# Autonomous-Drone-Racing-Lab/Efficient-Path-Planner

Hardware: AMD Instinct MI355X
Metric: validity checks/sec + full plan ms/track, 1/2/4/8 MI355X vs CPU ref (higher is better)
Workload: dtype f64; 1 GPU; C2: 1 track, 8 gates, 64 OBBs, 1,048,576 sampled states per step; obbs=64, can_pass_gate=False, parallelism=replicas x1 (independent samplers), process_group=solo, launch=hip graph of the K steps

## Files before the change

### efficient-path-planner_amd/csrc/epp_internal.h

```cpp
#pragma once
#include <math.h>
#include <stdint.h>

#include <mutex>
#include <shared_mutex>
#include <string>
#include <vector>

#include <hip/hip_runtime_api.h>

#include "epp.h"

namespace epp {
epp_status generate_trajectory_into(const double* wp, int32_t n_wp, const double* times, double v_max,
                                    double a_max, double dt, double t0, const double v0[3], const double a0[3],
                                    double* (*alloc)(void*, int64_t), void* ctx, int64_t* n_rows);
struct FusedCheck {
    const epp_world* world;
    const double* xyz;
    int64_t n;
    double min_distance;
    uint8_t* valid;
};
epp_status check_and_generate_into(const FusedCheck* chk, const double* wp, int32_t n_wp, const double* times,
// ... 20 lines not shown
                       int32_t* radj, uint16_t* radj16, void* stream);
epp_status check_knn_motions_rows(const epp_world* world, const double* nodes, int32_t* rows32, const int32_t* ids32,
                                  const int64_t* rows_n, int32_t cap, int32_t k, int32_t can_pass_gate,
                                  uint8_t* valid, uint16_t* out16, int32_t target, int64_t* count, void* stream,
                                  const MotionMask* marks = nullptr);
bool knn_motions_rows_supported(const epp_world* world);

struct PlanSeg {
    uint64_t seed;
    double s[3], g[3];
    double bound;
    double gbound;
    double glo[3], ghi[3];
    double h;
    int64_t row_off;
    int64_t need_off;
    int32_t cap;
    int32_t need_cap;
};
enum : int { kPbRows = 1, kPbPerSeg = 3 };
struct PlanBatchLayout {
    int32_t S = 0, k = 0, ns_log = 0, nbc = 0, cap_total = 0, nctr = 0;
    int64_t ns = 0, NS = 0, need_cap = 0;
    size_t o_seg = 0, o_ctr = 0, o_xyz = 0, o_valid = 0, o_nodes = 0, o_cstat = 0, o_kws = 0, kws_stride = 0,
           o_query = 0, o_ids32 = 0, o_rows32 = 0, o_rows16 = 0, o_ev = 0, o_mark = 0, o_map = 0, o_nstat = 0,
           o_need = 0, dev_bytes = 0;
    size_t h_seg = 0, h_hdr = 0, h_slot = 0, h_rows = 0, h_need = 0, h_done = 0, host_bytes = 0;
    int32_t done_n = 0;
};
PlanBatchLayout plan_batch_layout(int32_t S, int64_t ns, int32_t k, PlanSeg* segs);
void plan_batch_trace_print();
epp_status plan_batch_launch(const epp_world* world, int32_t can_pass_gate, const double lo[3], const double hi[3],
                             const PlanBatchLayout& L, void* dev, void* host, uint32_t seq, void* stream);
}

namespace epp {

enum Field : int {
    F_LOX = 0, F_LOY, F_LOZ, F_HIX, F_HIY, F_HIZ,
    F_CX, F_CY, F_CZ,
    F_COS, F_SIN,
    F_HX, F_HY, F_HZ,
    EPP_NF
};

constexpr int kRecDoubles = 17;
constexpr int R_META = 16;

constexpr int kPtDoubles = 16;
constexpr int P_TX = F_HX, P_TY = F_HY, P_TZ = F_HZ;
#if defined(__HIPCC__)
__host__ __device__
#endif
constexpr uint32_t pt_chunk_off(uint32_t i, uint32_t c) { return (i << 7) + ((c ^ ((i >> 1) & 7u)) << 4); }
constexpr uint32_t kIdFill = 0x8000u;

// ... 143 lines not shown
```

### efficient-path-planner_amd/csrc/host_plan_solve.cpp

```cpp
#include <atomic>
#include <chrono>
#include <condition_variable>
#include <cstdlib>
#include <cstring>
#include <deque>
#include <exception>
#include <functional>
#include <iostream>
#include <mutex>
#include <thread>

#include <hip/hip_runtime_api.h>
#include <immintrin.h>

#include "completion.h"
#include "graph_search.h"
#include "host_scratch.h"
#include "plan_solve.h"

namespace epp {

namespace {
using Clock = std::chrono::steady_clock;
double ms_between(Clock::time_point a, Clock::time_point b) { return std::chrono::duration<double, std::milli>(b - a).count(); }
// ... 44 lines not shown
        if (dev) epp_free(dev);
        dev = nullptr;
        cap = 0;
        check(epp_malloc(&dev, bytes), what);
        cap = bytes;
    }
    void ensure(size_t dev_bytes, size_t host_bytes) {
        if (dev_bytes > dcap_) regrow(dev_, dcap_, std::max(dev_bytes, dcap_ + dcap_ / 2), "planner batch workspace");
        if (host_bytes > host_.cap &&
            host_.grow(std::max(host_bytes, host_.cap + host_.cap / 2), true) != hipSuccess)
            throw std::runtime_error("planner batch: hipHostMalloc failed");
    }
    void* dev() const { return dev_; }
    char* host() const { return host_.as<char>(); }
    uint32_t next_seq() { return epp::next_seq(seq_); }
    struct Area {
        void* dev = nullptr;
        PinnedBuf pin;
        void* stream = nullptr;
        size_t dcap = 0;
        bool cold = true;
    };
    static size_t r256(size_t b) { return (b + 255) & ~size_t(255); }
    static size_t area_dev_bytes(int64_t n, int k) {
        const size_t m = (size_t)n * k;
        return r256(16) + r256(m * 4) + r256(m * 2) + r256(m) + r256((size_t)epp_knn_workspace_size((int32_t)n)) +
               3 * r256((size_t)(n + 1) * 4) + r256(m * 4) + r256(m * 2);
    }
    static size_t area_pin_bytes(int64_t n, int k) {
        return r256(64) + r256((size_t)n * 24) + r256((size_t)n * k * 4) + r256((size_t)(n + 1) * 4) +
               r256((size_t)n * k * 4);
    }
    void ensure_areas(size_t W, int64_t n, int k) {
        if (areas_.size() < W) areas_.resize(W);
        const size_t db = area_dev_bytes(n, k), pb = area_pin_bytes(n, k);
        for (size_t w = 0; w < W; ++w) {
            Area& a = areas_[w];
            if (!a.stream) check(epp_stream_create(&a.stream), "stream");
            if (db > a.dcap) regrow(a.dev, a.dcap, db, "planner fallback workspace");
            if (pb > a.pin.cap) {
                if (a.pin.grow(pb) != hipSuccess) throw std::runtime_error("planner fallback: hipHostMalloc failed");
                check(epp_memcpy_d2h_async(a.pin.p, a.dev, std::min(pb, a.dcap), a.stream), "planner fallback warm-up");
                check(epp_stream_sync(a.stream), "planner fallback warm-up");
            }
        }
    }
    Area& area(size_t w) { return areas_[w]; }
    void* stream() {
        if (!stream_) check(epp_stream_create(&stream_), "stream");
        return stream_;
    }
    ~BatchScratch() {
        if (dev_) epp_free(dev_);
        if (stream_) epp_stream_destroy(stream_);
        for (Area& a : areas_) {
            if (a.dev) epp_free(a.dev);
            if (a.stream) epp_stream_destroy(a.stream);
        }
// ... 29 lines not shown
        rev.fill.assign(16384, 0);
        rev.radj.assign((size_t)16384 * k, 0);
        ss.begin(16384);
        ss.heap.resize(ss.heap.capacity() / 4);
        ss.heap.clear();
    }
};

bool plan_trace() {
    static const bool t = [] {
        const char* e = std::getenv("EPP_PLAN_TRACE");
        return e && std::atoi(e) == 1;
    }();
    return t;
}

class WholeTable {
public:
    struct Counts {
        int64_t kept, into_goal;
    };
    WholeTable(const PlanContext& c, BatchScratch::Area& a, ProblemOut& o) : c_(c), a_(a), o_(o) {}

    void enqueue(const double* d_nodes, int32_t n, const double box[6], bool want_counts = false) {
        t0_ = mark_ = Clock::now();
        const int k = c_.k;
        d_nodes_ = d_nodes;
        n_ = n;
        m_ = (size_t)n * k;
        narrow_ = n <= 65535;
        const size_t ws_bytes = (size_t)epp_knn_workspace_size(n);
        if (BatchScratch::area_dev_bytes(n, k) > a_.dcap || BatchScratch::area_pin_bytes(n, k) > a_.pin.cap)
            throw std::runtime_error("planPath: fallback workspace too small");
        char* dp = static_cast<char*>(a_.dev);
        d_ecnt_ = reinterpret_cast<int64_t*>(dp);
        d_nbr_ = reinterpret_cast<int32_t*>(dp + r256(16));
        d_nbr16_ = narrow_ ? reinterpret_cast<uint16_t*>(reinterpret_cast<char*>(d_nbr_) + r256(m_ * 4)) : nullptr;
        uint8_t* d_ev = reinterpret_cast<uint8_t*>(d_nbr_) + r256(m_ * 4) + r256(m_ * 2);
        d_ws_ = d_ev + r256(m_);
        void* st = a_.stream;
        if (hipMemsetAsync(d_ecnt_, 0, 16, static_cast<hipStream_t>(st)) != hipSuccess)
            throw std::runtime_error("planPath: clearing the edge counts failed");
        check(epp_knn_ws_box(d_nodes, n, k, 0.0, box, box + 3, d_nbr_, d_ws_, ws_bytes, st), "knn");
        const int32_t cp = c_.canPass ? 1 : 0;
        const epp_status ks = check_knn_motions_masked(c_.world, d_nodes, d_nbr_, n, k, cp, d_ev, d_nbr16_, 1, d_ecnt_, st);
        if (ks == EPP_ERR_UNSUPPORTED) {
            ThreadScratch& ts = ThreadScratch::get();
            ts.reset(2 * ThreadScratch::rounded(m_ * 24));
            double* d_e1 = static_cast<double*>(ts.carve(m_ * 24));
            double* d_e2 = static_cast<double*>(ts.carve(m_ * 24));
            check(epp_knn_edges(d_nodes, d_nbr_, n, k, d_e1, d_e2, st), "edges");
            check(epp_check_motions(c_.world, d_e1, d_e2, (int64_t)m_, cp, 0, d_ev, st), "motion check");
            check(mask_edges_count_acc(d_nbr_, d_ev, (int64_t)m_, 1, d_ecnt_, st, d_nbr16_), "mask edges");
        } else {
            check(ks, "motion check");
        }
        if (want_counts) check(epp_memcpy_d2h_async(ecnt(), d_ecnt_, 16, st), "download");
// ... 93 lines not shown

struct Emitted {
    const uint64_t* hdr;
    const uint32_t* slots;
    const uint16_t* rows;
    const double* need;
    std::vector<int64_t> first;
    int S, k;
    const double* d_nodes0;
    size_t node_stride;
    int64_t hv(int field, int p) const { return (int64_t)hdr[kPbPerSeg + field * S + p]; }
    const double* d_nodes(int p) const { return d_nodes0 + (size_t)p * node_stride * 3; }
};

int rows_symmetrised(SolveScratch& sc, const Rows& g, double bound, ProblemOut& o) {
    sc.rev.build(g);
    const Searched s = search_rows(sc.ss, g, NodePos{sc.ndc.data()}, bound, &sc.rev);
    o.pops += s.pops;
    o.why = s.r == -1 ? 5 : s.r == 0 ? 6 : -1;
    o.symmetrised = s.r == 1 ? 1 : 0;
    return s.r;
}

void census(int p, double bound, const Rows& g, WholeTable& wt, ProblemOut& o) {
    SolveScratch& sc = SolveScratch::get();
    o.fallback = 1;
    o.why = 2;
    const auto ts0 = Clock::now();
    const int r2 = rows_symmetrised(sc, g, bound, o);
    if (plan_trace())
        std::cerr << "[plan trace] problem " << p << ": symmetrised search on " << o.restricted_rows << " rows / "
                  << g.m << " nodes: " << o.pops << " closed, " << ms_between(ts0, Clock::now()) << " ms, result " << r2
                  << " (copies before: " << o.ms_restricted << " ms)" << std::endl;
    const WholeTable::Counts cnt = wt.counts();
    if (cnt.into_goal > 0) o.why = 2;
    if (cnt.into_goal == 0 && r2 == 1) {
        o.path = extract_path(sc.ss, NodePos{sc.ndc.data()});
        o.found = true;
        o.fallback = 0;
        o.census = 1;
        o.rows_down = o.restricted_rows;
    } else {
        o.found = wt.search(o.path);
        o.rows_down = o.n;
        o.symmetrised = 0;
    }
}

void solve_problem(const Emitted& em, int p, const PlanSeg& seg, const double* kbox, WholeTable& wt, ProblemOut& o) {
    const int k = em.k;
    const int64_t n = em.hv(3, p);
    o.n = n;
    const int64_t packed = em.hv(0, p);
    const int64_t m = std::min<int64_t>(em.hv(4, p), seg.need_cap);
    const auto t0 = Clock::now();
    int r = 0;
    if (seg.cap > 0) o.why = (n > 65535 || packed > seg.cap || m < 2) ? 0 : em.hv(5, p) != 0 ? 1 : -1;
    if (seg.cap > 0 && n <= 65535 && packed <= seg.cap && em.hv(5, p) == 0 && m >= 2) {
        const int64_t first = em.first[p], nrow = em.first[p + 1] - first;
        SolveScratch& sc = SolveScratch::get();
        grow_to(sc.ndc, (size_t)m * 3, 3 * 16384);
        grow_to(sc.rowc, (size_t)nrow * k, (size_t)16384 * k);
        std::memcpy(sc.ndc.data(), em.need + 3 * seg.need_off, (size_t)m * 24);
        std::memcpy(sc.rowc.data(), em.rows + (size_t)first * k, (size_t)nrow * k * 2);
        o.ms_copy = ms_between(t0, Clock::now());
        grow_to(sc.row_of, (size_t)m, 16384);
        std::fill(sc.row_of.begin(), sc.row_of.begin() + m, -1);
        for (int64_t sl = 0; sl < nrow; ++sl) sc.row_of[em.slots[first + sl] & 0xFFFFu] = (int32_t)sl;
        const Rows g{sc.rowc.data(), sc.row_of.data(), k, m};
        const NodePos pos{sc.ndc.data()};
        const bool goal_edges = em.hv(2, p) > 0;
        const Searched fwd = goal_edges ? search_rows(sc.ss, g, pos, seg.bound) : Searched{-1, 0};
        r = fwd.r;
        o.restricted_rows = packed;
        o.pops = fwd.pops;
        o.nodes = m;
        o.why = r == -1 ? 3 : r == 0 ? 4 : -1;
        if (r == 0) {
            r = rows_symmetrised(sc, g, seg.bound, o);
        } else if (!goal_edges) {
            o.ms_restricted = ms_between(t0, Clock::now());
            o.ms_search += o.ms_restricted;
            wt.enqueue(em.d_nodes(p), (int32_t)n, kbox, true);
            census(p, seg.bound, g, wt, o);
            return;
        }
        if (r == 1) {
            o.path = extract_path(sc.ss, pos);
            o.found = true;
            o.edges_checked = packed * k;
            o.edges_valid = em.hv(1, p);
            o.rows_down = packed;
        }
    }
    o.ms_restricted = ms_between(t0, Clock::now());
    o.ms_search += o.ms_restricted;
    if (r != 1) {
        o.fallback = seg.cap > 0 ? 1 : 0;
        wt.enqueue(em.d_nodes(p), (int32_t)n, kbox);
        o.found = wt.search(o.path);
        o.rows_down += n;
    }
}

template <class Solve>
class SolveCrew {
public:
    SolveCrew(size_t W, int S, int k, Solve& solve) : S_(S), k_(k), solve_(solve), err_(S), pending_(W - 1) {
        int devno = 0;
        if (hipGetDevice(&devno) != hipSuccess) devno = 0;
        for (size_t t = 1; t < W; ++t) plan_pool().submit([this, devno, t] { wait_then_drain(devno, t); });
    }
    ~SolveCrew() {
        if (go_.load(std::memory_order_acquire) == 0) set_go(-1);
        join();
    }
    void run() {
        set_go(1);
        drain(0);
        join();
        for (const auto& e : err_)
            if (e) std::rethrow_exception(e);
    }

// ... 79 lines not shown
    const size_t W = std::min((size_t)S, (size_t)std::max(1, c.threads));
    bs.ensure_areas(W, nmax, k);
    char* H = bs.host();
    std::memcpy(H + L.h_seg, segs.data(), sizeof(PlanSeg) * S);
    Emitted em{reinterpret_cast<const uint64_t*>(H + L.h_hdr), reinterpret_cast<const uint32_t*>(H + L.h_slot),
               reinterpret_cast<const uint16_t*>(H + L.h_rows), reinterpret_cast<const double*>(H + L.h_need),
               std::vector<int64_t>(S + 1, 0), S, k,
               reinterpret_cast<const double*>(static_cast<const char*>(bs.dev()) + L.o_nodes), (size_t)L.NS};
    BatchSolution sol;
    sol.out.resize(S);
    auto solve = [&](int p, size_t w) {
        WholeTable wt(c, bs.area(w), sol.out[p]);
        solve_problem(em, p, segs[p], kbox[p].data(), wt, sol.out[p]);
    };
    SolveCrew<decltype(solve)> crew(W, S, k, solve);
    sol.ms_enqueue = launch_and_wait(c, L, bs, t0);
    for (int p = 0; p < S; ++p) em.first[p + 1] = em.first[p] + std::min<int64_t>(em.hv(0, p), segs[p].cap);
    for (size_t a = 0; a < W; ++a) {
        BatchScratch::Area& ar = bs.area(a);
        if (!ar.cold) continue;
        ar.cold = false;
        ProblemOut unused;
        WholeTable wt(c, ar, unused);
        wt.enqueue(em.d_nodes(0), (int32_t)em.hv(3, 0), kbox[0].data());
        (void)wt.search(unused.path);
    }
    sol.ms_batch = ms_between(t0, Clock::now());
    crew.run();
    return sol;
}

}
```

### efficient-path-planner_amd/csrc/plan_batch.hip

```cpp
#include <hip/hip_runtime.h>

#include <algorithm>
#include <cstdio>
#include <cstdlib>
#include <string>

#include "completion.h"
#include "epp_internal.h"
#include "knn_grid.h"

namespace epp {
namespace {

constexpr int kPbSegSmall = 16;
struct PlanBatchDev {
    const PlanSeg* seg;
    const PlanSeg* seg_h;
    uint64_t seeds[kPbSegSmall];
    int32_t caps[kPbSegSmall];
    int S, k, ns_log, nbc, cap_total, nctr;
    int64_t ns, NS;
    double lo[3], hi[3];
    double* xyz;
    uint8_t* valid;
    double* nodes;
    unsigned long long* cstat;
    unsigned long long* nstat;
    unsigned long long* ctr;
    char* kws;
    size_t kws_stride, l_cell, l_sidx, l_sxyz, l_cnt, l_start, l_fill, l_stat;
    int l_cap, nclr;
    int32_t* query;
    int32_t* ids32;
    int32_t* rows32;
    uint16_t* rows16;
    uint8_t* mark;
    int32_t* map;
    double* need;
};

struct KnnSeg {
    KnnGrid* g;
    int* cell_of;
    int* sidx;
    double* sxyz;
    int* cnt;
    int* start;
    int* fill;
    unsigned long long* stat;
};
__device__ __forceinline__ KnnSeg knn_seg(const PlanBatchDev& P, int p) {
    char* b = P.kws + (size_t)p * P.kws_stride;
    return {reinterpret_cast<KnnGrid*>(b), reinterpret_cast<int*>(b + P.l_cell), reinterpret_cast<int*>(b + P.l_sidx),
            reinterpret_cast<double*>(b + P.l_sxyz), reinterpret_cast<int*>(b + P.l_cnt),
            reinterpret_cast<int*>(b + P.l_start), reinterpret_cast<int*>(b + P.l_fill),
            reinterpret_cast<unsigned long long*>(b + P.l_stat)};
}
__device__ __forceinline__ unsigned long long& pb_ctr(const PlanBatchDev& P, int field, int p) {
    return P.ctr[kPbPerSeg + field * P.S + p];
}
enum : int { kFQueries = 0, kFKept = 1, kFGoal = 2, kFNodes = 3, kFNeed = 4, kFInexact = 5 };

static_assert(sizeof(PlanSeg) % 8 == 0, "PlanSeg copied as 8-byte words");

__global__ __launch_bounds__(256) void k_pb_sample(PlanBatchDev P) {
    const int p = blockIdx.y;
    const int64_t i = (int64_t)blockIdx.x * 256 + threadIdx.x;
    const bool small = P.seg_h != nullptr;
    if (small && blockIdx.x == 0 && threadIdx.x < (int)(sizeof(PlanSeg) / 8))
        reinterpret_cast<uint64_t*>(const_cast<PlanSeg*>(P.seg) + p)[threadIdx.x] =
            reinterpret_cast<const uint64_t*>(P.seg_h + p)[threadIdx.x];
    if (i < P.nbc) P.cstat[(int64_t)p * P.nbc + i] = 0ull;
    if (P.cap_total > 0 && i < P.NS / kCompactChunk) P.nstat[(int64_t)p * (P.NS / kCompactChunk) + i] = 0ull;
    if (P.cap_total > 0 && i < (P.NS >> 4))
        reinterpret_cast<uint4*>(P.mark + ((int64_t)p << P.ns_log))[i] = make_uint4(0u, 0u, 0u, 0u);
    if (p == 0 && i < P.nctr) P.ctr[i] = 0ull;
    const uint64_t seed = small ? P.seeds[p] : P.seg[p].seed;
    const int32_t cap = small ? P.caps[p] : P.seg[p].cap;
    if (cap > 0) {
        const KnnSeg ks = knn_seg(P, p);
        if (i < P.nclr) ks.cnt[i] = 0;
        if (i == 0) {
            const PlanSeg q = small ? P.seg_h[p] : P.seg[p];
            KnnGrid gv{};
            int64_t cells = 1;
            double h = q.h;
            for (;;) {
                cells = 1;
                for (int d = 0; d < 3; ++d) {
                    gv.dims[d] = (int)fmin((q.ghi[d] - q.glo[d]) / h, 1023.0) + 1;
                    cells *= gv.dims[d];
                }
                if (cells <= P.l_cap) break;
                h *= 1.25;
            }
            for (int d = 0; d < 3; ++d) gv.lo[d] = q.glo[d];
            gv.h = h;
            gv.inv_h = 1.0 / h;
            gv.ncell = (int)cells;
            gv.qbound = 1e300;
            *ks.g = gv;
        }
    }
    if (i >= P.ns) return;
    sample_uniform(seed, (uint64_t)i, P.lo, P.hi, P.xyz + ((int64_t)p * P.ns + i) * 3);
}

__device__ __forceinline__ double pb_ellipse(const PlanSeg& q, const double* x) {
    const double ds = sqrt((x[0] - q.s[0]) * (x[0] - q.s[0]) + (x[1] - q.s[1]) * (x[1] - q.s[1]) +
                           (x[2] - q.s[2]) * (x[2] - q.s[2]));
    const double dg = sqrt((x[0] - q.g[0]) * (x[0] - q.g[0]) + (x[1] - q.g[1]) * (x[1] - q.g[1]) +
                           (x[2] - q.g[2]) * (x[2] - q.g[2]));
    return ds + dg;
}

__device__ __forceinline__ bool pb_member(const PlanBatchDev& P, const PlanSeg& q, const KnnSeg& ks, const KnnGrid& g,
                                          int p, int node, const double* x) {
    const double f = pb_ellipse(q, x);
    int c = -1;
    if (f <= q.gbound) {
        const int cx = knn_cell_axis(x[0], g, 0), cy = knn_cell_axis(x[1], g, 1), cz = knn_cell_axis(x[2], g, 2);
        c = (cz * g.dims[1] + cy) * g.dims[0] + cx;
        atomicAdd(&ks.cnt[c], 1);
    }
    ks.cell_of[node] = c;
    return f <= q.bound * (1.0 + 1e-8) + 1e-6;
}

__global__ __launch_bounds__(kCompactThreads) void k_pb_compact(PlanBatchDev P, uint32_t tag) {
    const int p = blockIdx.y, b = blockIdx.x, nb = gridDim.x;
    double* out = P.nodes + (int64_t)p * P.NS * 3;
    const PlanSeg& q = P.seg[p];
    const bool R = q.cap > 0;
    const KnnSeg ks = knn_seg(P, p);
    KnnGrid g{};
    if (R) g = *ks.g;
    const double* xyz = P.xyz + (int64_t)p * P.ns * 3;
    const uint8_t* valid = P.valid + (int64_t)p * P.ns;
    unsigned long long* st = P.cstat + (int64_t)p * P.nbc;
    constexpr int NW = kCompactThreads / 64;
    __shared__ int wcnt[kCompactRounds * NW];
    __shared__ int qcnt[NW];
    __shared__ long long s_excl;
    __shared__ unsigned long long s_qbase;
    const int lane = threadIdx.x & 63, wv = threadIdx.x >> 6;
    bool inq2 = false;
    if (b == 0 && threadIdx.x < 2) {
        const double* e = threadIdx.x == 0 ? q.s : q.g;
        out[3 * threadIdx.x] = e[0];
        out[3 * threadIdx.x + 1] = e[1];
        out[3 * threadIdx.x + 2] = e[2];
        if (R) inq2 = pb_member(P, q, ks, g, p, (int)threadIdx.x, e);
    }
    const int64_t i0 = (int64_t)b * kCompactChunk + threadIdx.x;
    bool v[kCompactRounds];
    unsigned long long bal[kCompactRounds];
#pragma unroll
    for (int r = 0; r < kCompactRounds; ++r) {
        const int64_t i = i0 + r * kCompactThreads;
        v[r] = i < P.ns && valid[i] != 0;
    }
#pragma unroll
    for (int r = 0; r < kCompactRounds; ++r) {
        bal[r] = __ballot(v[r]);
        if (lane == 0) wcnt[r * NW + wv] = __popcll(bal[r]);
    }
    __syncthreads();
    int before[kCompactRounds], total = 0;
#pragma unroll
    for (int qq = 0; qq < kCompactRounds * NW; ++qq) {
#pragma unroll
        for (int r = 0; r < kCompactRounds; ++r)
            if (qq == r * NW + wv) before[r] = total;
        total += wcnt[qq];
    }
    if (wv == 0) {
        if (lane == 0) lb_publish(st, b, tag, b == 0, total);
        const long long ex = b == 0 ? 0ll : lb_exclusive(st, b, tag);
        if (lane == 0) {
            if (b > 0) lb_publish(st, b, tag, true, ex + total);
            s_excl = ex;
            if (b == nb - 1) pb_ctr(P, kFNodes, p) = (unsigned long long)(ex + total + 2);
        }
    }
    __syncthreads();
    const long long ex = s_excl;
    bool inq[kCompactRounds];
    int node[kCompactRounds];
#pragma unroll
    for (int r = 0; r < kCompactRounds; ++r) {
        inq[r] = false;
        node[r] = 0;
        if (v[r]) {
            const int64_t i = i0 + r * kCompactThreads;
            const int64_t at = 2 + ex + before[r] +
                               (int64_t)__builtin_amdgcn_mbcnt_hi((uint32_t)(bal[r] >> 32),
                                                                  __builtin_amdgcn_mbcnt_lo((uint32_t)bal[r], 0u));
            const double x[3] = {xyz[3 * i], xyz[3 * i + 1], xyz[3 * i + 2]};
            out[3 * at] = x[0];
            out[3 * at + 1] = x[1];
            out[3 * at + 2] = x[2];
            node[r] = (int)at;
            if (R) inq[r] = pb_member(P, q, ks, g, p, (int)at, x);
        }
    }
    if (!R) return;
    unsigned long long qb[kCompactRounds + 1];
    int wq = 0;
#pragma unroll
    for (int r = 0; r < kCompactRounds; ++r) {
        qb[r] = __ballot(inq[r]);
        wq += __popcll(qb[r]);
    }
    qb[kCompactRounds] = __ballot(inq2);
    wq += __popcll(qb[kCompactRounds]);
    if (lane == 0) qcnt[wv] = wq;
    __syncthreads();
    if (threadIdx.x == 0) {
        int t = 0;
        for (int w = 0; w < NW; ++w) t += qcnt[w];
        s_qbase = t ? atomicAdd(&pb_ctr(P, kFQueries, p), (unsigned long long)t) : 0ull;
    }
    __syncthreads();
    unsigned long long rnk = s_qbase;
    for (int w = 0; w < wv; ++w) rnk += qcnt[w];
    const unsigned long long below = (1ull << lane) - 1ull;
#pragma unroll
    for (int r = 0; r <= kCompactRounds; ++r) {
        const bool mine = r < kCompactRounds ? inq[r] : inq2;
        const int nd = r < kCompactRounds ? node[r] : (int)threadIdx.x;
        if (mine) {
            const unsigned long long at = rnk + __popcll(qb[r] & below);
            if (at < (unsigned long long)q.cap) P.query[q.row_off + (int64_t)at] = nd;
        }
        rnk += __popcll(qb[r]);
    }
}

__global__ __launch_bounds__(kScanThreads) void k_pb_knn_scan(PlanBatchDev P, uint32_t tag) {
    if (P.seg[blockIdx.y].cap <= 0) return;
    const KnnSeg ks = knn_seg(P, blockIdx.y);
    knn_scan_block(ks.g, ks.cnt, ks.start, ks.stat, tag, blockIdx.x);
}

__global__ __launch_bounds__(256) void k_pb_knn_scatter(PlanBatchDev P) {
    const int p = blockIdx.y;
    if (P.seg[p].cap <= 0) return;
    const int i = blockIdx.x * 256 + threadIdx.x;
    if (i >= (int)pb_ctr(P, kFNodes, p)) return;
    const KnnSeg ks = knn_seg(P, p);
    const int c = ks.cell_of[i];
    if (c < 0) return;
    const int pos = ks.start[c] + atomicAdd(&ks.fill[c], 1);
    if (pos >= ks.start[c + 1]) return;
    const double* nd = P.nodes + ((int64_t)p * P.NS + i) * 3;
    ks.sidx[pos] = i;
    ks.sxyz[3 * pos] = nd[0];
    ks.sxyz[3 * pos + 1] = nd[1];
    ks.sxyz[3 * pos + 2] = nd[2];
}

#ifdef EPP_PB_ROWS_TL
constexpr int kPbTl = 1 << 15;
__device__ unsigned long long g_pb_rows_tl[kPbTl][6];
#define EPP_PBTL(d, k, v)                                                     \
    do {                                                                      \
        if ((threadIdx.x & 63) == 0 && (d) < kPbTl) g_pb_rows_tl[(d)][(k)] = (v); \
    } while (0)
#define EPP_PBTL_NOW() __builtin_amdgcn_s_memrealtime()
#else
#define EPP_PBTL(d, k, v) \
    do {                  \
// ... 371 lines not shown
    int64_t rows = 0, need = 0;
    for (int p = 0; p < S; ++p) {
        segs[p].cap = std::max(0, segs[p].cap);
        segs[p].row_off = rows;
        rows += segs[p].cap;
        segs[p].need_off = need;
        segs[p].need_cap =
            segs[p].cap > 0 ? (int32_t)((std::min<int64_t>((int64_t)segs[p].cap * (k + 1) + 2, ns + 2) + 1) & ~1ll) : 0;
        need += segs[p].need_cap;
    }
    L.cap_total = (int32_t)rows;
    L.need_cap = need;
    L.nctr = kPbPerSeg + 6 * S;
    const bool R = rows > 0;
    const KnnLayout kl = knn_layout((int)(ns + 2));
    size_t o = 0;
    auto take = [&](size_t bytes) {
        const size_t at = o;
        o += al(bytes);
        return at;
    };
    L.o_seg = take((size_t)S * sizeof(PlanSeg));
    L.o_ctr = take((size_t)L.nctr * 8);
    L.o_xyz = take((size_t)S * ns * 24);
    L.o_valid = take((size_t)S * ns);
    L.o_nodes = take((size_t)S * L.NS * 24);
    L.o_cstat = take((size_t)S * L.nbc * 8);
    L.kws_stride = R ? al(kl.bytes) : 0;
    L.o_kws = take((size_t)S * L.kws_stride);
    const size_t capr = ((size_t)rows + 3) & ~size_t(3);
    L.o_query = take(capr * 4);
    L.o_ids32 = take(capr * 4);
    L.o_rows32 = take(capr * k * 4);
    L.o_rows16 = take(capr * k * 2);
    L.o_ev = take(capr * k);
    L.o_mark = take(R ? (size_t)S * L.NS : 0);
    L.o_map = take(R ? (size_t)S * L.NS * 4 : 0);
    L.o_nstat = take(R ? (size_t)S * (L.NS / kCompactChunk) * 8 : 0);
    L.o_need = take((size_t)L.need_cap * 24 + 16);
    L.dev_bytes = o;
    o = 0;
    L.h_seg = take((size_t)S * sizeof(PlanSeg));
    L.h_hdr = take((size_t)L.nctr * 8);
    L.h_slot = take(capr * 4);
    L.h_rows = take(capr * k * 2);
    L.h_need = take((size_t)L.need_cap * 24 + 16);
    {
        static const int eb = [] {
// ... 33 lines not shown
    t.name[t.n] = name;
    (void)hipEventRecord(t.ev[t.n++], s);
}
}

void epp::plan_batch_trace_print() {
    PbTrace& t = pb_trace();
    if (!t.on || t.n < 2) return;
    (void)hipEventSynchronize(t.ev[t.n - 1]);
    std::string line = "pb_trace:";
    float tot = 0;
    for (int i = 1; i < t.n; ++i) {
        float ms = 0;
        (void)hipEventElapsedTime(&ms, t.ev[i - 1], t.ev[i]);
        tot += ms;
        line += std::string(" ") + t.name[i] + "=" + std::to_string((int)(ms * 1000.0f + 0.5f));
    }
    line += " total=" + std::to_string((int)(tot * 1000.0f + 0.5f));
    std::fprintf(stderr, "%s\n", line.c_str());
    t.n = 0;
}

epp_status epp::plan_batch_launch(const epp_world* world, int32_t can_pass_gate, const double lo[3], const double hi[3],
                                  const PlanBatchLayout& L, void* dev, void* host, uint32_t seq, void* stream) {
    if (!world || !dev || !host || L.S < 1 || L.S > 64 || L.ns < 1 || (L.k != 4 && L.k != 8 && L.k != 16) ||
        ((int64_t)L.S << L.ns_log) >= (1ll << 31) || (reinterpret_cast<uintptr_t>(dev) & 255) ||
        (reinterpret_cast<uintptr_t>(host) & 255)) {
        set_error("plan_batch_launch: invalid argument");
        return EPP_ERR_INVALID_ARGUMENT;
    }
    char* d = static_cast<char*>(dev);
    char* h = static_cast<char*>(host);
    hipStream_t s = static_cast<hipStream_t>(stream);
    const KnnLayout kl = knn_layout((int)(L.ns + 2));
    PlanBatchDev P{};
    P.seg = reinterpret_cast<const PlanSeg*>(d + L.o_seg);
    P.S = L.S;
    P.k = L.k;
    P.ns_log = L.ns_log;
    P.nbc = L.nbc;
    P.cap_total = L.cap_total;
    P.nctr = L.nctr;
    P.ns = L.ns;
    P.NS = L.NS;
    for (int i = 0; i < 3; ++i) {
        P.lo[i] = lo[i];
        P.hi[i] = hi[i];
    }
    P.xyz = reinterpret_cast<double*>(d + L.o_xyz);
    P.valid = reinterpret_cast<uint8_t*>(d + L.o_valid);
    P.nodes = reinterpret_cast<double*>(d + L.o_nodes);
    P.cstat = reinterpret_cast<unsigned long long*>(d + L.o_cstat);
    P.ctr = reinterpret_cast<unsigned long long*>(d + L.o_ctr);
    P.kws = d + L.o_kws;
    P.kws_stride = L.kws_stride;
    P.l_cell = kl.cell;
    P.l_sidx = kl.sidx;
    P.l_sxyz = kl.sxyz;
    P.l_cnt = kl.cnt;
    P.l_start = kl.start;
    P.l_fill = kl.fill;
    P.l_stat = kl.stat;
    P.l_cap = kl.cap;
    P.nclr = (int)((kl.start - kl.cnt) / sizeof(int));
    P.query = reinterpret_cast<int32_t*>(d + L.o_query);
    P.ids32 = reinterpret_cast<int32_t*>(d + L.o_ids32);
    P.rows32 = reinterpret_cast<int32_t*>(d + L.o_rows32);
    P.rows16 = reinterpret_cast<uint16_t*>(d + L.o_rows16);
    P.mark = reinterpret_cast<uint8_t*>(d + L.o_mark);
    P.nstat = reinterpret_cast<unsigned long long*>(d + L.o_nstat);
    P.map = reinterpret_cast<int32_t*>(d + L.o_map);
    P.need = reinterpret_cast<double*>(d + L.o_need);
    const unsigned S = (unsigned)L.S;
    const bool R = L.cap_total > 0;
    P.seg_h = nullptr;
    if (L.S <= kPbSegSmall) {
        P.seg_h = reinterpret_cast<const PlanSeg*>(h + L.h_seg);
        for (int p = 0; p < L.S; ++p) {
            P.seeds[p] = P.seg_h[p].seed;
            P.caps[p] = P.seg_h[p].cap;
        }
    } else {
        if (hipMemcpyAsync(d + L.o_seg, h + L.h_seg, (size_t)L.S * sizeof(PlanSeg), hipMemcpyHostToDevice, s) !=
            hipSuccess)
            return last("plan_batch_launch");
    }
    const int64_t clr = std::max<int64_t>({L.ns, R ? L.NS >> 4 : 0, R ? (int64_t)P.nclr : 0, (int64_t)L.nbc, (int64_t)L.nctr});
    pb_mark(s, "begin");
    hipLaunchKernelGGL(k_pb_sample, dim3((unsigned)((clr + 255) / 256), S), dim3(256), 0, s, P);
    if (const epp_status st = epp_check_states(world, P.xyz, (int64_t)L.S * L.ns, can_pass_gate, P.valid, nullptr,
                                               nullptr, stream))
        return st;
    pb_mark(s, "states");
    hipLaunchKernelGGL(k_pb_compact, dim3((unsigned)L.nbc, S), dim3(kCompactThreads), 0, s, P, next_scan_tag());
    if (R) {
        const unsigned gn = (unsigned)((L.ns + 2 + 255) / 256);
        pb_mark(s, "compact_member");
        hipLaunchKernelGGL(k_pb_knn_scan, dim3((unsigned)kl.scan_blocks, S), dim3(kScanThreads), 0, s, P, next_scan_tag());
        hipLaunchKernelGGL(k_pb_knn_scatter, dim3(gn, S), dim3(256), 0, s, P);
        pb_mark(s, "scan_scatter");
        static const int rows_wg = [] {
            const char* e = std::getenv("EPP_PB_ROWS_WG");
            const int v = e && *e ? std::atoi(e) : 28;
            return std::max(1, std::min(64, v));
        }();
        const dim3 gr((unsigned)std::max(1, cu_count_planner() * rows_wg)), br(64);
        if (L.k == 4) hipLaunchKernelGGL(k_pb_rows<4>, gr, br, 0, s, P);
        else if (L.k == 8) hipLaunchKernelGGL(k_pb_rows<8>, gr, br, 0, s, P);
        else hipLaunchKernelGGL(k_pb_rows<16>, gr, br, 0, s, P);
        pb_mark(s, "rows");
        MotionMask marks;
        marks.mark = P.mark;
        marks.pkept = P.ctr + kPbPerSeg + kFKept * L.S;
        marks.pgoal = P.ctr + kPbPerSeg + kFGoal * L.S;
        marks.ns_log = L.ns_log;
        marks.nprob = L.S;
        if (const epp_status st = check_knn_motions_rows(
                world, P.nodes, P.rows32, P.ids32, reinterpret_cast<const int64_t*>(P.ctr + kPbRows), L.cap_total,
                L.k, can_pass_gate, reinterpret_cast<uint8_t*>(d + L.o_ev), P.rows16, -1, nullptr, stream, &marks))
            return st;
// ... 13 lines not shown
```

### efficient-path-planner_amd/csrc/planner.hip

```cpp
#include <hip/hip_runtime.h>

#include <algorithm>
#include <atomic>
#include <mutex>
#include <string>

#include "cached_ws.h"
#include "epp_internal.h"
#include "planner_common.h"

namespace epp {

namespace {
std::atomic<uint32_t> g_scan_tag{0};
}
uint32_t next_scan_tag() {
    uint32_t t;
    do t = (g_scan_tag.fetch_add(1, std::memory_order_relaxed) + 1u) & 0xffffffu;
    while (t == 0u);
    return t;
}

int cu_count_planner() {
    int dev = 0, cus = 256;
// ... 78 lines not shown
            if (b == nb - 1) *n_out = ex + total + add;
        }
    }
    __syncthreads();
    const long long ex = s_excl;
#pragma unroll
    for (int r = 0; r < kCompactRounds; ++r) {
        if (v[r]) {
            const int64_t i = i0 + r * kCompactThreads;
            const int64_t p = ex + before[r] +
                              (int64_t)__builtin_amdgcn_mbcnt_hi((uint32_t)(bal[r] >> 32),
                                                                 __builtin_amdgcn_mbcnt_lo((uint32_t)bal[r], 0u));
            out[3 * p] = xyz[3 * i];
            out[3 * p + 1] = xyz[3 * i + 1];
            out[3 * p + 2] = xyz[3 * i + 2];
        }
    }
}
__global__ __launch_bounds__(kCompactThreads) void k_compact(const double* __restrict__ xyz,
                                                             const uint8_t* __restrict__ valid, int64_t n,
                                                             unsigned long long* __restrict__ st, uint32_t tag,
                                                             double* __restrict__ out, int64_t* __restrict__ n_out) {
    compact_block(xyz, valid, n, st, tag, out, n_out, 0, blockIdx.x, gridDim.x);
}

__global__ void k_mask_edges(int32_t* __restrict__ nbr, const uint8_t* __restrict__ valid, int64_t m) {
    const int64_t e = (int64_t)blockIdx.x * blockDim.x + threadIdx.x;
    if (e < m && !valid[e]) nbr[e] = -1;
}

constexpr int kMaskThreads = 1024;
__global__ __launch_bounds__(kMaskThreads) void k_mask_edges_count(int32_t* __restrict__ nbr,
                                                                   const uint8_t* __restrict__ valid, int64_t m,
                                                                   int32_t target,
                                                                   unsigned long long* __restrict__ count,
                                                                   uint16_t* __restrict__ out16) {
    __shared__ uint32_t part[2][kMaskThreads / 64];
    uint32_t c = 0, ci = 0;
    for (int64_t e = (int64_t)blockIdx.x * kMaskThreads + threadIdx.x; e < m;
         e += (int64_t)gridDim.x * kMaskThreads) {
        const int32_t v = nbr[e];
        const bool ok = valid[e] != 0;
        if (!ok) nbr[e] = -1;
        const bool keep = ok && v >= 0;
        if (out16) out16[e] = keep ? (uint16_t)v : (uint16_t)0xFFFF;
        c += keep ? 1u : 0u;
// ... 173 lines not shown
    const int64_t blocks = std::min<int64_t>((m + kMaskThreads - 1) / kMaskThreads, 256);
    hipLaunchKernelGGL(k_mask_edges_count, dim3((unsigned)blocks), dim3(kMaskThreads), 0, s, nbr, valid, m, target,
                       reinterpret_cast<unsigned long long*>(count), out16);
    return last("epp_mask_edges_count");
}

extern "C" {

epp_status epp_knn_edges(const double* nodes, const int32_t* nbr, int32_t n, int32_t k, double* s1,
                         double* s2, void* stream) {
    if (n < 0 || k <= 0 || (n > 0 && (!nodes || !nbr || !s1 || !s2))) {
        set_error("epp_knn_edges: invalid argument");
        return EPP_ERR_INVALID_ARGUMENT;
    }
    const int64_t m = (int64_t)n * k;
    if (m == 0) return EPP_OK;
    hipLaunchKernelGGL(k_knn_edges, dim3((unsigned)((m + 255) / 256)), dim3(256), 0, (hipStream_t)stream, nodes,
                       nbr, m, k, s1, s2);
    return last("epp_knn_edges");
}

}

epp_status epp::reverse_csr(const int32_t* nbr, int32_t n, int32_t k, int32_t* cnt, int32_t* fill, int32_t* roff,
                            int32_t* radj, uint16_t* radj16, void* stream) {
    if (n <= 0 || k <= 0 || !nbr || !cnt || !fill || !roff || !radj) {
        set_error("reverse_csr: invalid argument");
        return EPP_ERR_INVALID_ARGUMENT;
    }
    hipStream_t s = static_cast<hipStream_t>(stream);
    const int64_t m = (int64_t)n * k;
    if (hipMemsetAsync(cnt, 0, (size_t)n * 4, s) != hipSuccess) return last("reverse_csr");
    hipLaunchKernelGGL(k_rev_count, dim3((unsigned)((m + 255) / 256)), dim3(256), 0, s, nbr, m, cnt);
    hipLaunchKernelGGL(k_rev_scan, dim3(1), dim3(1024), 0, s, cnt, n, roff, fill);
    hipLaunchKernelGGL(k_rev_fill, dim3((unsigned)((m + 255) / 256)), dim3(256), 0, s, nbr, m, k, fill, radj);
    hipLaunchKernelGGL(k_rev_sort, dim3((unsigned)((n + 255) / 256)), dim3(256), 0, s, roff, n, radj, radj16);
    return last("reverse_csr");
}
```

Before: 151.5 billion state validity checks/s.

## Fuse sampling, ellipse prefilter and collision check into the batch front kernel

The separate sample kernel, the generic state-check pass and the compaction kernel are replaced by a single front kernel. It generates samples in registers, rejects those outside the informed ellipse bound before classifying them, runs the OBB hit tests inline, and then compacts the survivors. This removes the xyz and valid buffers, their global memory traffic and two launches, and skips collision work for samples outside the ellipse. The trade-off is higher register pressure in the fused kernel. The fallback path now rebuilds the node table on demand through a new helper, which adds a host sync on that path.

```diff
diff --git a/efficient-path-planner_amd/csrc/epp_internal.h b/efficient-path-planner_amd/csrc/epp_internal.h
--- a/efficient-path-planner_amd/csrc/epp_internal.h
+++ b/efficient-path-planner_amd/csrc/epp_internal.h
@@ -66,7 +66,7 @@
 struct PlanBatchLayout {
     int32_t S = 0, k = 0, ns_log = 0, nbc = 0, cap_total = 0, nctr = 0;
     int64_t ns = 0, NS = 0, need_cap = 0;
-    size_t o_seg = 0, o_ctr = 0, o_xyz = 0, o_valid = 0, o_nodes = 0, o_cstat = 0, o_kws = 0, kws_stride = 0,
+    size_t o_seg = 0, o_ctr = 0, o_nodes = 0, o_cstat = 0, o_kws = 0, kws_stride = 0,
            o_query = 0, o_ids32 = 0, o_rows32 = 0, o_rows16 = 0, o_ev = 0, o_mark = 0, o_map = 0, o_nstat = 0,
            o_need = 0, dev_bytes = 0;
     size_t h_seg = 0, h_hdr = 0, h_slot = 0, h_rows = 0, h_need = 0, h_done = 0, host_bytes = 0;
@@ -75,7 +75,12 @@
 PlanBatchLayout plan_batch_layout(int32_t S, int64_t ns, int32_t k, PlanSeg* segs);
 void plan_batch_trace_print();
 epp_status plan_batch_launch(const epp_world* world, int32_t can_pass_gate, const double lo[3], const double hi[3],
-                             const PlanBatchLayout& L, void* dev, void* host, uint32_t seq, void* stream);
+                             const PlanBatchLayout& L, void* dev, void* host, uint32_t seq, void* stream,
+                             bool front_only = false);
+size_t node_table_ws_bytes(int64_t ns);
+epp_status node_table_build(const epp_world* world, uint64_t seed, const double lo[3], const double hi[3], int64_t ns,
+                            const double s[3], const double g[3], int32_t can_pass_gate, double* nodes,
+                            int64_t* n_out, void* ws, void* stream);
 }
 
 namespace epp {
diff --git a/efficient-path-planner_amd/csrc/host_plan_solve.cpp b/efficient-path-planner_amd/csrc/host_plan_solve.cpp
--- a/efficient-path-planner_amd/csrc/host_plan_solve.cpp
+++ b/efficient-path-planner_amd/csrc/host_plan_solve.cpp
@@ -90,10 +90,13 @@
         bool cold = true;
     };
     static size_t r256(size_t b) { return (b + 255) & ~size_t(255); }
-    static size_t area_dev_bytes(int64_t n, int k) {
+    static size_t area_build_bytes(int64_t nmax) {
+        return r256((size_t)nmax * 24) + r256(8) + r256(node_table_ws_bytes(std::max<int64_t>(1, nmax - 2)));
+    }
+    static size_t area_dev_bytes(int64_t n, int k, int64_t nmax) {
         const size_t m = (size_t)n * k;
-        return r256(16) + r256(m * 4) + r256(m * 2) + r256(m) + r256((size_t)epp_knn_workspace_size((int32_t)n)) +
-               3 * r256((size_t)(n + 1) * 4) + r256(m * 4) + r256(m * 2);
+        return area_build_bytes(nmax) + r256(16) + r256(m * 4) + r256(m * 2) + r256(m) +
+               r256((size_t)epp_knn_workspace_size((int32_t)n)) + 3 * r256((size_t)(n + 1) * 4) + r256(m * 4) + r256(m * 2);
     }
     static size_t area_pin_bytes(int64_t n, int k) {
         return r256(64) + r256((size_t)n * 24) + r256((size_t)n * k * 4) + r256((size_t)(n + 1) * 4) +
@@ -101,7 +104,7 @@
     }
     void ensure_areas(size_t W, int64_t n, int k) {
         if (areas_.size() < W) areas_.resize(W);
-        const size_t db = area_dev_bytes(n, k), pb = area_pin_bytes(n, k);
+        const size_t db = area_dev_bytes(n, k, n), pb = area_pin_bytes(n, k);
         for (size_t w = 0; w < W; ++w) {
             Area& a = areas_[w];
             if (!a.stream) check(epp_stream_create(&a.stream), "stream");
@@ -177,17 +180,40 @@
     };
     WholeTable(const PlanContext& c, BatchScratch::Area& a, ProblemOut& o) : c_(c), a_(a), o_(o) {}
 
-    void enqueue(const double* d_nodes, int32_t n, const double box[6], bool want_counts = false) {
-        t0_ = mark_ = Clock::now();
+    int32_t enqueue_built(const PlanSeg& seg, const double box[6], bool want_counts = false) {
+        const auto t0 = Clock::now();
+        const int64_t nmax = c_.box.nmax;
+        if (BatchScratch::area_build_bytes(nmax) > a_.dcap || a_.pin.cap < r256(64))
+            throw std::runtime_error("planPath: fallback workspace too small");
+        char* dp = static_cast<char*>(a_.dev);
+        double* d_nodes = reinterpret_cast<double*>(dp);
+        int64_t* d_n = reinterpret_cast<int64_t*>(dp + r256((size_t)nmax * 24));
+        void* ws = dp + r256((size_t)nmax * 24) + r256(8);
+        void* st = a_.stream;
+        check(node_table_build(c_.world, seg.seed, c_.box.lo, c_.box.hi, nmax - 2, seg.s, seg.g, c_.canPass ? 1 : 0,
+                               d_nodes, d_n, ws, st),
+              "node table");
+        int64_t* h_n = a_.pin.as<int64_t>() + 2;
+        check(epp_memcpy_d2h_async(h_n, d_n, 8, st), "download");
+        check(epp_stream_sync(st), "sync");
+        const int32_t n = (int32_t)*h_n;
+        if (n < 2 || n > nmax) throw std::runtime_error("planPath: the fallback's node table has an impossible size");
+        enqueue(d_nodes, n, box, want_counts, &t0);
+        return n;
+    }
+
+    void enqueue(const double* d_nodes, int32_t n, const double box[6], bool want_counts = false,
+                 const Clock::time_point* started = nullptr) {
+        t0_ = mark_ = started ? *started : Clock::now();
         const int k = c_.k;
         d_nodes_ = d_nodes;
         n_ = n;
         m_ = (size_t)n * k;
         narrow_ = n <= 65535;
         const size_t ws_bytes = (size_t)epp_knn_workspace_size(n);
-        if (BatchScratch::area_dev_bytes(n, k) > a_.dcap || BatchScratch::area_pin_bytes(n, k) > a_.pin.cap)
+        if (BatchScratch::area_dev_bytes(n, k, c_.box.nmax) > a_.dcap || BatchScratch::area_pin_bytes(n, k) > a_.pin.cap)
             throw std::runtime_error("planPath: fallback workspace too small");
-        char* dp = static_cast<char*>(a_.dev);
+        char* dp = static_cast<char*>(a_.dev) + BatchScratch::area_build_bytes(c_.box.nmax);
         d_ecnt_ = reinterpret_cast<int64_t*>(dp);
         d_nbr_ = reinterpret_cast<int32_t*>(dp + r256(16));
         d_nbr16_ = narrow_ ? reinterpret_cast<uint16_t*>(reinterpret_cast<char*>(d_nbr_) + r256(m_ * 4)) : nullptr;
@@ -327,7 +353,7 @@
     return s.r;
 }
 
-void census(int p, double bound, const Rows& g, WholeTable& wt, ProblemOut& o) {
+void census(int p, double bound, const Rows& g, WholeTable& wt, int64_t n_all, ProblemOut& o) {
     SolveScratch& sc = SolveScratch::get();
     o.fallback = 1;
     o.why = 2;
@@ -347,7 +373,7 @@
         o.rows_down = o.restricted_rows;
     } else {
         o.found = wt.search(o.path);
-        o.rows_down = o.n;
+        o.rows_down = n_all;
         o.symmetrised = 0;
     }
 }
@@ -360,6 +386,11 @@
     const int64_t m = std::min<int64_t>(em.hv(4, p), seg.need_cap);
     const auto t0 = Clock::now();
     int r = 0;
+    auto whole_table = [&](bool want_counts) -> int64_t {
+        if (seg.cap > 0) return wt.enqueue_built(seg, kbox, want_counts);
+        wt.enqueue(em.d_nodes(p), (int32_t)n, kbox, want_counts);
+        return n;
+    };
     if (seg.cap > 0) o.why = (n > 65535 || packed > seg.cap || m < 2) ? 0 : em.hv(5, p) != 0 ? 1 : -1;
     if (seg.cap > 0 && n <= 65535 && packed <= seg.cap && em.hv(5, p) == 0 && m >= 2) {
         const int64_t first = em.first[p], nrow = em.first[p + 1] - first;
@@ -386,8 +417,8 @@
         } else if (!goal_edges) {
             o.ms_restricted = ms_between(t0, Clock::now());
             o.ms_search += o.ms_restricted;
-            wt.enqueue(em.d_nodes(p), (int32_t)n, kbox, true);
-            census(p, seg.bound, g, wt, o);
+            const int64_t n_all = whole_table(true);
+            census(p, seg.bound, g, wt, n_all, o);
             return;
         }
         if (r == 1) {
@@ -402,9 +433,9 @@
     o.ms_search += o.ms_restricted;
     if (r != 1) {
         o.fallback = seg.cap > 0 ? 1 : 0;
-        wt.enqueue(em.d_nodes(p), (int32_t)n, kbox);
+        const int64_t n_all = whole_table(false);
         o.found = wt.search(o.path);
-        o.rows_down += n;
+        o.rows_down += n_all;
     }
 }
 
@@ -530,7 +561,8 @@
         ar.cold = false;
         ProblemOut unused;
         WholeTable wt(c, ar, unused);
-        wt.enqueue(em.d_nodes(0), (int32_t)em.hv(3, 0), kbox[0].data());
+        if (segs[0].cap > 0) wt.enqueue_built(segs[0], kbox[0].data());
+        else wt.enqueue(em.d_nodes(0), (int32_t)em.hv(3, 0), kbox[0].data());
         (void)wt.search(unused.path);
     }
     sol.ms_batch = ms_between(t0, Clock::now());
diff --git a/efficient-path-planner_amd/csrc/plan_batch.hip b/efficient-path-planner_amd/csrc/plan_batch.hip
--- a/efficient-path-planner_amd/csrc/plan_batch.hip
+++ b/efficient-path-planner_amd/csrc/plan_batch.hip
@@ -5,6 +5,7 @@
 #include <cstdlib>
 #include <string>
 
+#include "collision_common.h"
 #include "completion.h"
 #include "epp_internal.h"
 #include "knn_grid.h"
@@ -16,13 +17,10 @@
 struct PlanBatchDev {
     const PlanSeg* seg;
     const PlanSeg* seg_h;
-    uint64_t seeds[kPbSegSmall];
     int32_t caps[kPbSegSmall];
     int S, k, ns_log, nbc, cap_total, nctr;
     int64_t ns, NS;
     double lo[3], hi[3];
-    double* xyz;
-    uint8_t* valid;
     double* nodes;
     unsigned long long* cstat;
     unsigned long long* nstat;
@@ -63,7 +61,7 @@
 
 static_assert(sizeof(PlanSeg) % 8 == 0, "PlanSeg copied as 8-byte words");
 
-__global__ __launch_bounds__(256) void k_pb_sample(PlanBatchDev P) {
+__global__ __launch_bounds__(256) void k_pb_clear(PlanBatchDev P) {
     const int p = blockIdx.y;
     const int64_t i = (int64_t)blockIdx.x * 256 + threadIdx.x;
     const bool small = P.seg_h != nullptr;
@@ -72,10 +70,7 @@
             reinterpret_cast<const uint64_t*>(P.seg_h + p)[threadIdx.x];
     if (i < P.nbc) P.cstat[(int64_t)p * P.nbc + i] = 0ull;
     if (P.cap_total > 0 && i < P.NS / kCompactChunk) P.nstat[(int64_t)p * (P.NS / kCompactChunk) + i] = 0ull;
-    if (P.cap_total > 0 && i < (P.NS >> 4))
-        reinterpret_cast<uint4*>(P.mark + ((int64_t)p << P.ns_log))[i] = make_uint4(0u, 0u, 0u, 0u);
     if (p == 0 && i < P.nctr) P.ctr[i] = 0ull;
-    const uint64_t seed = small ? P.seeds[p] : P.seg[p].seed;
     const int32_t cap = small ? P.caps[p] : P.seg[p].cap;
     if (cap > 0) {
         const KnnSeg ks = knn_seg(P, p);
@@ -102,8 +97,6 @@
             *ks.g = gv;
         }
     }
-    if (i >= P.ns) return;
-    sample_uniform(seed, (uint64_t)i, P.lo, P.hi, P.xyz + ((int64_t)p * P.ns + i) * 3);
 }
 
 __device__ __forceinline__ double pb_ellipse(const PlanSeg& q, const double* x) {
@@ -114,9 +107,8 @@
     return ds + dg;
 }
 
-__device__ __forceinline__ bool pb_member(const PlanBatchDev& P, const PlanSeg& q, const KnnSeg& ks, const KnnGrid& g,
-                                          int p, int node, const double* x) {
-    const double f = pb_ellipse(q, x);
+__device__ __forceinline__ bool pb_member(const PlanSeg& q, const KnnSeg& ks, const KnnGrid& g, int node,
+                                          const double* x, double f) {
     int c = -1;
     if (f <= q.gbound) {
         const int cx = knn_cell_axis(x[0], g, 0), cy = knn_cell_axis(x[1], g, 1), cz = knn_cell_axis(x[2], g, 2);
@@ -127,7 +119,7 @@
     return f <= q.bound * (1.0 + 1e-8) + 1e-6;
 }
 
-__global__ __launch_bounds__(kCompactThreads) void k_pb_compact(PlanBatchDev P, uint32_t tag) {
+__global__ __launch_bounds__(kCompactThreads) void k_pb_front(PlanBatchDev P, WorldView w, int can_pass, uint32_t tag) {
     const int p = blockIdx.y, b = blockIdx.x, nb = gridDim.x;
     double* out = P.nodes + (int64_t)p * P.NS * 3;
     const PlanSeg& q = P.seg[p];
@@ -135,8 +127,7 @@
     const KnnSeg ks = knn_seg(P, p);
     KnnGrid g{};
     if (R) g = *ks.g;
-    const double* xyz = P.xyz + (int64_t)p * P.ns * 3;
-    const uint8_t* valid = P.valid + (int64_t)p * P.ns;
+    const Acc a = make_acc(w.blob, w.blob, w);
     unsigned long long* st = P.cstat + (int64_t)p * P.nbc;
     constexpr int NW = kCompactThreads / 64;
     __shared__ int wcnt[kCompactRounds * NW];
@@ -150,15 +141,40 @@
         out[3 * threadIdx.x] = e[0];
         out[3 * threadIdx.x + 1] = e[1];
         out[3 * threadIdx.x + 2] = e[2];
-        if (R) inq2 = pb_member(P, q, ks, g, p, (int)threadIdx.x, e);
+        if (R) inq2 = pb_member(q, ks, g, (int)threadIdx.x, e, pb_ellipse(q, e));
     }
     const int64_t i0 = (int64_t)b * kCompactChunk + threadIdx.x;
+    const uint64_t seed = q.seed;
     bool v[kCompactRounds];
+    double x[kCompactRounds][3], f[kCompactRounds];
     unsigned long long bal[kCompactRounds];
 #pragma unroll
     for (int r = 0; r < kCompactRounds; ++r) {
         const int64_t i = i0 + r * kCompactThreads;
-        v[r] = i < P.ns && valid[i] != 0;
+        v[r] = i < P.ns;
+        f[r] = 0.0;
+        sample_uniform(seed, (uint64_t)i, P.lo, P.hi, x[r]);
+        if (R) {
+            f[r] = pb_ellipse(q, x[r]);
+            v[r] = v[r] && f[r] <= q.gbound;
+        }
+    }
+    const double* recs = reinterpret_cast<const double*>(w.blob + w.off_aos);
+    uint32_t cst[kCompactRounds], cn[kCompactRounds], cmax = 0;
+#pragma unroll
+    for (int r = 0; r < kCompactRounds; ++r) {
+        const uint32_t c = classify(a, w, x[r][0], x[r][1], x[r][2], cst[r]);
+        cn[r] = v[r] ? c : 0u;
+        cmax = max(cmax, cn[r]);
+    }
+    for (uint32_t j = 0; j < cmax; ++j) {
+#pragma unroll
+        for (int r = 0; r < kCompactRounds; ++r)
+            if (j < cn[r] && rec_hit<false>(recs + (size_t)a.co[cst[r] + j] * kRecDoubles, w.r_gate, w.r_obst, x[r][0],
+                                            x[r][1], x[r][2], can_pass != 0, 0.0)) {
+                v[r] = false;
+                cn[r] = 0u;
+            }
     }
 #pragma unroll
     for (int r = 0; r < kCompactRounds; ++r) {
@@ -192,16 +208,14 @@
         inq[r] = false;
         node[r] = 0;
         if (v[r]) {
-            const int64_t i = i0 + r * kCompactThreads;
             const int64_t at = 2 + ex + before[r] +
                                (int64_t)__builtin_amdgcn_mbcnt_hi((uint32_t)(bal[r] >> 32),
                                                                   __builtin_amdgcn_mbcnt_lo((uint32_t)bal[r], 0u));
-            const double x[3] = {xyz[3 * i], xyz[3 * i + 1], xyz[3 * i + 2]};
-            out[3 * at] = x[0];
-            out[3 * at + 1] = x[1];
-            out[3 * at + 2] = x[2];
+            out[3 * at] = x[r][0];
+            out[3 * at + 1] = x[r][1];
+            out[3 * at + 2] = x[r][2];
             node[r] = (int)at;
-            if (R) inq[r] = pb_member(P, q, ks, g, p, (int)at, x);
+            if (R) inq[r] = pb_member(q, ks, g, (int)at, x[r], f[r]);
         }
     }
     if (!R) return;
@@ -218,12 +232,12 @@
     __syncthreads();
     if (threadIdx.x == 0) {
         int t = 0;
-        for (int w = 0; w < NW; ++w) t += qcnt[w];
+        for (int w2 = 0; w2 < NW; ++w2) t += qcnt[w2];
         s_qbase = t ? atomicAdd(&pb_ctr(P, kFQueries, p), (unsigned long long)t) : 0ull;
     }
     __syncthreads();
     unsigned long long rnk = s_qbase;
-    for (int w = 0; w < wv; ++w) rnk += qcnt[w];
+    for (int w2 = 0; w2 < wv; ++w2) rnk += qcnt[w2];
     const unsigned long long below = (1ull << lane) - 1ull;
 #pragma unroll
     for (int r = 0; r <= kCompactRounds; ++r) {
@@ -247,7 +261,9 @@
     const int p = blockIdx.y;
     if (P.seg[p].cap <= 0) return;
     const int i = blockIdx.x * 256 + threadIdx.x;
-    if (i >= (int)pb_ctr(P, kFNodes, p)) return;
+    const int n = (int)pb_ctr(P, kFNodes, p);
+    if (16 * i < n) reinterpret_cast<uint4*>(P.mark + ((int64_t)p << P.ns_log))[i] = make_uint4(0u, 0u, 0u, 0u);
+    if (i >= n) return;
     const KnnSeg ks = knn_seg(P, p);
     const int c = ks.cell_of[i];
     if (c < 0) return;
@@ -665,8 +681,6 @@
     };
     L.o_seg = take((size_t)S * sizeof(PlanSeg));
     L.o_ctr = take((size_t)L.nctr * 8);
-    L.o_xyz = take((size_t)S * ns * 24);
-    L.o_valid = take((size_t)S * ns);
     L.o_nodes = take((size_t)S * L.NS * 24);
     L.o_cstat = take((size_t)S * L.nbc * 8);
     L.kws_stride = R ? al(kl.bytes) : 0;
@@ -746,7 +760,8 @@
 }
 
 epp_status epp::plan_batch_launch(const epp_world* world, int32_t can_pass_gate, const double lo[3], const double hi[3],
-                                  const PlanBatchLayout& L, void* dev, void* host, uint32_t seq, void* stream) {
+                                  const PlanBatchLayout& L, void* dev, void* host, uint32_t seq, void* stream,
+                                  bool front_only) {
     if (!world || !dev || !host || L.S < 1 || L.S > 64 || L.ns < 1 || (L.k != 4 && L.k != 8 && L.k != 16) ||
         ((int64_t)L.S << L.ns_log) >= (1ll << 31) || (reinterpret_cast<uintptr_t>(dev) & 255) ||
         (reinterpret_cast<uintptr_t>(host) & 255)) {
@@ -771,8 +786,6 @@
         P.lo[i] = lo[i];
         P.hi[i] = hi[i];
     }
-    P.xyz = reinterpret_cast<double*>(d + L.o_xyz);
-    P.valid = reinterpret_cast<uint8_t*>(d + L.o_valid);
     P.nodes = reinterpret_cast<double*>(d + L.o_nodes);
     P.cstat = reinterpret_cast<unsigned long long*>(d + L.o_cstat);
     P.ctr = reinterpret_cast<unsigned long long*>(d + L.o_ctr);
@@ -800,26 +813,26 @@
     P.seg_h = nullptr;
     if (L.S <= kPbSegSmall) {
         P.seg_h = reinterpret_cast<const PlanSeg*>(h + L.h_seg);
-        for (int p = 0; p < L.S; ++p) {
-            P.seeds[p] = P.seg_h[p].seed;
-            P.caps[p] = P.seg_h[p].cap;
-        }
+        for (int p = 0; p < L.S; ++p) P.caps[p] = P.seg_h[p].cap;
     } else {
         if (hipMemcpyAsync(d + L.o_seg, h + L.h_seg, (size_t)L.S * sizeof(PlanSeg), hipMemcpyHostToDevice, s) !=
             hipSuccess)
             return last("plan_batch_launch");
     }
-    const int64_t clr = std::max<int64_t>({L.ns, R ? L.NS >> 4 : 0, R ? (int64_t)P.nclr : 0, (int64_t)L.nbc, (int64_t)L.nctr});
+    const int64_t clr = std::max<int64_t>({R ? L.NS / kCompactChunk : 0, R ? (int64_t)P.nclr : 0, (int64_t)L.nbc, (int64_t)L.nctr});
     pb_mark(s, "begin");
-    hipLaunchKernelGGL(k_pb_sample, dim3((unsigned)((clr + 255) / 256), S), dim3(256), 0, s, P);
-    if (const epp_status st = epp_check_states(world, P.xyz, (int64_t)L.S * L.ns, can_pass_gate, P.valid, nullptr,
-                                               nullptr, stream))
-        return st;
-    pb_mark(s, "states");
-    hipLaunchKernelGGL(k_pb_compact, dim3((unsigned)L.nbc, S), dim3(kCompactThreads), 0, s, P, next_scan_tag());
+    hipLaunchKernelGGL(k_pb_clear, dim3((unsigned)((clr + 255) / 256), S), dim3(256), 0, s, P);
+    pb_mark(s, "clear");
+    {
+        IndexLease ix;
+        if (const epp_status st = ensure_index(world, &ix)) return st;
+        hipLaunchKernelGGL(k_pb_front, dim3((unsigned)L.nbc, S), dim3(kCompactThreads), 0, s, P, ix.view, can_pass_gate,
+                           next_scan_tag());
+    }
+    pb_mark(s, "front");
+    if (front_only) return last("plan_batch_launch");
     if (R) {
         const unsigned gn = (unsigned)((L.ns + 2 + 255) / 256);
-        pb_mark(s, "compact_member");
         hipLaunchKernelGGL(k_pb_knn_scan, dim3((unsigned)kl.scan_blocks, S), dim3(kScanThreads), 0, s, P, next_scan_tag());
         hipLaunchKernelGGL(k_pb_knn_scatter, dim3(gn, S), dim3(256), 0, s, P);
         pb_mark(s, "scan_scatter");
diff --git a/efficient-path-planner_amd/csrc/planner.hip b/efficient-path-planner_amd/csrc/planner.hip
--- a/efficient-path-planner_amd/csrc/planner.hip
+++ b/efficient-path-planner_amd/csrc/planner.hip
@@ -124,6 +124,24 @@
                                                              unsigned long long* __restrict__ st, uint32_t tag,
                                                              double* __restrict__ out, int64_t* __restrict__ n_out) {
     compact_block(xyz, valid, n, st, tag, out, n_out, 0, blockIdx.x, gridDim.x);
+}
+
+struct Ends {
+    double s[3], g[3];
+};
+__global__ __launch_bounds__(kCompactThreads) void k_compact_ends(const double* __restrict__ xyz,
+                                                                  const uint8_t* __restrict__ valid, int64_t n,
+                                                                  unsigned long long* __restrict__ st, uint32_t tag,
+                                                                  Ends e, double* __restrict__ out,
+                                                                  int64_t* __restrict__ n_out) {
+    if (blockIdx.x == 0 && threadIdx.x == 0) {
+#pragma unroll
+        for (int d = 0; d < 3; ++d) {
+            out[d] = e.s[d];
+            out[3 + d] = e.g[d];
+        }
+    }
+    compact_block(xyz, valid, n, st, tag, out + 6, n_out, 2, blockIdx.x, gridDim.x);
 }
 
 __global__ void k_mask_edges(int32_t* __restrict__ nbr, const uint8_t* __restrict__ valid, int64_t m) {
@@ -343,6 +361,39 @@
 
 }
 
+namespace {
+size_t nt_r256(size_t b) { return (b + 255) & ~size_t(255); }
+}
+size_t epp::node_table_ws_bytes(int64_t ns) {
+    return nt_r256((size_t)epp_compact_workspace_size(ns)) + nt_r256((size_t)ns * 24) + nt_r256((size_t)ns);
+}
+
+epp_status epp::node_table_build(const epp_world* world, uint64_t seed, const double lo[3], const double hi[3],
+                                 int64_t ns, const double s[3], const double g[3], int32_t can_pass_gate,
+                                 double* nodes, int64_t* n_out, void* ws, void* stream) {
+    if (!world || ns < 1 || !lo || !hi || !s || !g || !nodes || !n_out || !ws || (reinterpret_cast<uintptr_t>(ws) & 255)) {
+        set_error("node_table_build: invalid argument");
+        return EPP_ERR_INVALID_ARGUMENT;
+    }
+    hipStream_t st = static_cast<hipStream_t>(stream);
+    char* w = static_cast<char*>(ws);
+    const int nb = (int)((ns + kCompactChunk - 1) / kCompactChunk);
+    unsigned long long* stat = reinterpret_cast<unsigned long long*>(w);
+    double* xyz = reinterpret_cast<double*>(w + nt_r256((size_t)epp_compact_workspace_size(ns)));
+    uint8_t* valid = reinterpret_cast<uint8_t*>(reinterpret_cast<char*>(xyz) + nt_r256((size_t)ns * 24));
+    hipLaunchKernelGGL(k_sample_uniform, dim3((unsigned)((ns + 255) / 256)), dim3(256), 0, st, seed, lo[0], lo[1], lo[2],
+                       hi[0], hi[1], hi[2], ns, (int64_t)0, xyz, stat, (int64_t)nb);
+    if (const epp_status rc = epp_check_states(world, xyz, ns, can_pass_gate, valid, nullptr, nullptr, stream)) return rc;
+    Ends e;
+    for (int d = 0; d < 3; ++d) {
+        e.s[d] = s[d];
+        e.g[d] = g[d];
+    }
+    hipLaunchKernelGGL(k_compact_ends, dim3((unsigned)nb), dim3(kCompactThreads), 0, st, xyz, valid, ns, stat,
+                       next_scan_tag(), e, nodes, n_out);
+    return last("node_table_build");
+}
+
 epp_status epp::reverse_csr(const int32_t* nbr, int32_t n, int32_t k, int32_t* cnt, int32_t* fill, int32_t* roff,
                             int32_t* radj, uint16_t* radj16, void* stream) {
     if (n <= 0 || k <= 0 || !nbr || !cnt || !fill || !roff || !radj) {
```

Result: no change. 151.1 billion state validity checks/s (-0.2%).
